# bikuta6/nbody-deep-sim

Measured on AMD Instinct MI355X. Metric: pair-interactions/sec, direct O(N^2) leapfrog N-body, fp32, higher is better.
Workload: dtype f32; 1 GPU; Plummer sphere, 65536 particles, direct all-pairs leapfrog step (BASELINE configs[1] shape: 65536 bodies per GPU); n_particles=65536, particles_per_gpu=65536, seed=1234, parallelism=single GPU

## Files before the change

include/nbd.h:

```cpp
#ifndef NBD_H_
#define NBD_H_

#include <stddef.h>
#include <stdint.h>

#ifdef __cplusplus
extern "C" {
#endif

#define NBD_ABI_VERSION 2
#define NBD_E_BADARG (-1)
#define NBD_E_WORKSPACE (-2)
#define NBD_E_UNSUPPORTED (-3)

#define NBD_SRC_PAD 64
#define NBD_CC_TILE 128
#define NBD_CC_GROUPS 8
#define NBD_CC_MAX_RES 4

typedef void* nbd_stream_t;

int nbd_abi_version(void);
size_t nbd_struct_size(const char* name);
const char* nbd_strerror(int code);
// ... 31 lines not shown
                                       float c_kick, void* workspace, size_t workspace_bytes, nbd_stream_t stream);

int nbd_kick_drift_f32(float* pos, float* vel, const float* acc, const float* mass, int n,
                       float c_kick, float c_drift, float* posm, nbd_stream_t stream);

int nbd_kick_f32(float* vel, const float* acc, int n, float c, nbd_stream_t stream);

int nbd_drift_f32(float* pos, const float* vel, int n, float c, nbd_stream_t stream);

int nbd_snapshot_f32(const float* pos, const float* vel, const float* acc, int n, float* out, nbd_stream_t stream);
int nbd_snapshot_f64(const double* pos, const double* vel, const double* acc, int n, double* out, nbd_stream_t stream);

size_t nbd_step_workspace_bytes(int n);

size_t nbd_step_workspace_pref_bytes(int n);

int nbd_leapfrog_step_f32(float* pos, float* vel, const float* acc_in, float* acc_out,
                          const float* mass, int n, float dt_half, float dt, float softening_sq,
                          float g_const, float* posm, void* workspace, size_t workspace_bytes,
                          nbd_stream_t stream);

int nbd_leapfrog_step_ev_f32(float* pos, float* vel, const float* acc_in, float* acc_out,
                             const float* mass, int n, float dt_half, float dt, float softening_sq,
                             float g_const, float* posm, void* workspace, size_t workspace_bytes,
                             nbd_stream_t stream, void* ev_force_begin, void* ev_force_end);
int nbd_leapfrog_step_uniform_f32(float* pos, float* vel, const float* acc_in, float* acc_out, const float* mass,
                                  float mass_value, int n, float dt_half, float dt, float softening_sq, float g_const,
                                  float* posm, void* workspace, size_t workspace_bytes, nbd_stream_t stream,
                                  void* ev_force_begin, void* ev_force_end);

size_t nbd_accel_sym_workspace_bytes(int n);
int nbd_accel_sym_uniform_f32(const float* posm, int n, float softening_sq, float g_const, float mass_value,
                              float* acc_out, void* workspace, size_t workspace_bytes, int variant, nbd_stream_t stream);

int nbd_euler_step_f32(float* pos, float* vel, float* acc_out, const float* mass, int n, float dt,
                       float softening_sq, float g_const, float* posm, void* workspace,
                       size_t workspace_bytes, nbd_stream_t stream);

size_t nbd_energy_workspace_bytes(int n);

int nbd_energy_f32(const float* posm, const float* vel, int n, float softening, float g_const,
                   double* out_uk, void* workspace, size_t workspace_bytes, nbd_stream_t stream);

size_t nbd_potential_workspace_bytes(int n_src, int n_tgt);
int nbd_potential_f32(const float* posm_src, int n_src, const float* posm_tgt, int n_tgt, int tgt_global_offset,
                      float softening_sq, float g_const, double* phi_out, void* workspace, size_t workspace_bytes,
                      nbd_stream_t stream);
int nbd_invariants_f64(const float* posm, const float* vel, const double* phi, int n, double* out_row,
                       nbd_stream_t stream);

int nbd_batch_plan(const int* offsets, int n_scenes, int* n_items, int* posm_rows, size_t* plan_bytes,
                   size_t* workspace_bytes);
int nbd_batch_plan_fill(const int* offsets, int n_scenes, void* plan, size_t plan_bytes);
int nbd_batch_pack_posm_f32(const int* offsets, int n_scenes, const void* plan, size_t plan_bytes, const float* pos,
                            const float* mass, float* posm, nbd_stream_t stream);
int nbd_batch_accel_f32(const int* offsets, int n_scenes, const void* plan, size_t plan_bytes, const float* pos,
                        const float* mass, const float* softening_sq, const float* g_const, float* acc_out,
                        float* posm, void* workspace, size_t workspace_bytes, nbd_stream_t stream);
int nbd_batch_leapfrog_step_f32(const int* offsets, int n_scenes, const void* plan, size_t plan_bytes, float* pos,
                                float* vel, const float* acc_in, float* acc_out, const float* mass, const float* dt_half,
                                const float* dt, const float* softening_sq, const float* g_const, float* posm,
                                void* workspace, size_t workspace_bytes, nbd_stream_t stream);
int nbd_batch_euler_step_f32(const int* offsets, int n_scenes, const void* plan, size_t plan_bytes, float* pos,
                             float* vel, float* acc_out, const float* mass, const float* dt, const float* softening_sq,
                             const float* g_const, float* posm, void* workspace, size_t workspace_bytes,
                             nbd_stream_t stream);
// ... 572 lines not shown
```

nbody-deep-sim_amd/csrc/direct_force.hip:

```cpp
#include <hip/hip_runtime.h>
#include <string.h>
#include <stdint.h>

#include <type_traits>

#include "../../include/nbd.h"
#include "direct_kernels.h"

namespace {

template <bool MASKED, int KU, bool UNI = false>
__global__ __launch_bounds__(64 * kWaves, KU == 4 ? 8 : 5) void accel_kernel(
    const f4* __restrict__ src, const SrcView sv, const f4* __restrict__ tgt,
    int n_tgt, int tgt_off, float eps2, float scale, float* __restrict__ out, int out_rows, int tile_len) {
  __shared__ f4 lds[kAccelLdsF4];
  const int tz = blockIdx.z * tile_len;
  const int t_base = blockIdx.x * kTgtPerWG;
  accel_body<KU, UNI>(src + tz, sv, std::integral_constant<bool, MASKED>{}, tgt + tz, n_tgt, tgt_off, t_base, blockIdx.y, eps2, scale, lds,
                      out + (size_t)tz * 3 + ((size_t)blockIdx.y * out_rows + t_base) * 3);
}

constexpr int kSymTile = 1024;
constexpr int kSymChunks = kSymTile / kChunk;
constexpr int kSymSlots = 16;
// ... 112 lines not shown
        const float v = (t & 1) ? v2.y : v2.x;
        float* o = o_own + t * 64 * 3 + comp;
        *o = init ? v : *o + v;
      }
    return;
  }
  __syncthreads();
  float* const mo = ldsf + (sg * 4 + tg) * 12 * 64;
#pragma unroll
  for (int t = 0; t < 4; ++t)
#pragma unroll
    for (int comp = 0; comp < 3; ++comp) {
      const f2 v2 = own[(t >> 1) * 3 + comp];
      mo[(comp * 4 + t) * 64 + lane] = (t & 1) ? v2.y : v2.x;
    }
  __syncthreads();
  if (sg != 0) return;
#pragma unroll
  for (int t = 0; t < 4; ++t)
#pragma unroll
    for (int comp = 0; comp < 3; ++comp) {
      const float* src = ldsf + tg * 12 * 64 + (comp * 4 + t) * 64 + lane;
      float v = src[0];
#pragma unroll
      for (int g = 1; g < SG; ++g) v += src[g * 4 * 12 * 64];
      float* o = o_own + t * 64 * 3 + comp;
      *o = init ? v : *o + v;
    }
}

constexpr int kSym2Pairs = kSymChunks / 2;
constexpr int kSym2T = 8;
constexpr int kSym2G = 2;

__global__ __launch_bounds__(512, 4) void accel_sym2_kernel(const f4* __restrict__ posm, int n, int m, int r0,
                                                            int n_slots, float eps2, float* __restrict__ out) {
  constexpr int kXyF = kSym2Pairs * 128 * 4;
  constexpr int kZF = kSym2Pairs * 128 * 2;
  constexpr int kReactF = 2 * 8 * 6 * 64;
  constexpr int kOwnF = 8 * 3 * kSym2T * 64;
  static_assert(kXyF + kZF + kReactF == kOwnF, "one 48-KiB LDS image");
  __shared__ f4 lds[kOwnF / 4];
  float* const ldsf = reinterpret_cast<float*>(lds);
  f4* const xy = lds;
  f2* const zz = reinterpret_cast<f2*>(ldsf + kXyF);
  float* const react = ldsf + kXyF + kZF;

  int ta, tb, slot;
  bool init;
  sym_round_match(blockIdx.x, m, r0, n_slots, ta, tb, slot, init);

  const int lane = threadIdx.x & 63;
  const int wave = __builtin_amdgcn_readfirstlane(threadIdx.x >> 6);
  const int tg = wave & 1, sg = wave >> 1;
  {
    const f4 u = posm[tb * kSymTile + wave * kChunk + lane];
    const f4 v = posm[tb * kSymTile + (wave + kSym2Pairs) * kChunk + lane];
    const f4 q = {u.x, v.x, u.y, v.y};
    const f2 z = {u.z, v.z};
    xy[wave * 128 + lane] = q; xy[wave * 128 + 64 + lane] = q;
    zz[wave * 128 + lane] = z; zz[wave * 128 + 64 + lane] = z;
  }
  const int row0 = ta * kSymTile + tg * 512 + lane;
  f2 txy[kSym2T], tzz[kSym2T / 2];
  f2 ax[kSym2T], ay[kSym2T], az[kSym2T];
#pragma unroll
  for (int t = 0; t < kSym2T; ++t) {
    const f4 q = posm[row0 + t * 64];
    txy[t] = f2{q.x, q.y};
    if (t & 1) tzz[t >> 1].y = q.z; else tzz[t >> 1].x = q.z;
    ax[t] = ay[t] = az[t] = f2{0.f, 0.f};
  }
  f2 e2 = {eps2, eps2};
  asm volatile("" : "+v"(e2));
  __syncthreads();

#pragma unroll 1
  for (int j = 0; j < 2; ++j) {
    const int p = sg * 2 + j;
    const f4* const bxy = xy + p * 128 + lane;
    const f2* const bz = zz + p * 128 + lane;
    f2 rx = {0.f, 0.f}, ry = {0.f, 0.f}, rz = {0.f, 0.f};
#pragma unroll 1
// ... 61 lines not shown
#pragma unroll
    for (int i = 0; i < 6; ++i) olda[i] = o_a[threadIdx.x + i * 512];
  }
  __syncthreads();

#pragma unroll
  for (int i = 0; i < 6; ++i) {
    const int o = threadIdx.x + i * 512;
    const int row = o / 3, comp = o - row * 3;
    const int c = row >> 6, l = row & 63, p = c & (kSym2Pairs - 1), hf = c / kSym2Pairs;
    const float* rs = react + ((p & 1) * 8 + (p >> 1) * 2) * 6 * 64 + (comp * 2 + hf) * 64 + l;
    const float v = rs[0] + rs[6 * 64];
    o_b[o] = init ? v : oldb[i] + v;
  }
  __syncthreads();
#pragma unroll
  for (int t = 0; t < kSym2T; ++t) {
    float* const mo = ldsf + ((sg * 2 + tg) * 3 * kSym2T + t) * 64 + lane;
    mo[0 * kSym2T * 64] = ax[t].x + ax[t].y;
    mo[1 * kSym2T * 64] = ay[t].x + ay[t].y;
    mo[2 * kSym2T * 64] = az[t].x + az[t].y;
  }
  __syncthreads();
#pragma unroll
  for (int i = 0; i < 6; ++i) {
    const int o = threadIdx.x + i * 512;
    const int row = o / 3, comp = o - row * 3;
    const int g = row >> 9, t = (row >> 6) & (kSym2T - 1), l = row & 63;
    const float* os = ldsf + ((g * 3 + comp) * kSym2T + t) * 64 + l;
    constexpr int kSg = 2 * 3 * kSym2T * 64;
    const float v = ((os[0] + os[kSg]) + os[2 * kSg]) + os[3 * kSg];
    o_a[o] = init ? v : olda[i] + v;
  }
}

__global__ __launch_bounds__(256) void finish_kernel(const float* __restrict__ slabs, int n_slabs,
                                                     size_t slab_stride, float g, float* __restrict__ acc,
                                                     float* __restrict__ vel, float c_kick, int n3) {
  __shared__ float part[4][64];
  const int lane = threadIdx.x & 63, w = threadIdx.x >> 6;
  const int i = blockIdx.x * 64 + lane;
  float sum = 0.f;
  if (i < n3)
    for (int s = w; s < n_slabs; s += 4) sum += slabs[s * slab_stride + i];
  part[w][lane] = sum;
  __syncthreads();
  if (w != 0 || i >= n3) return;
  const float a = __fmul_rn(g, (part[0][lane] + part[1][lane]) + (part[2][lane] + part[3][lane]));
  acc[i] = a;
  if (vel) vel[i] = __fadd_rn(vel[i], __fmul_rn(c_kick, a));
}

__global__ __launch_bounds__(256) void pack_kernel(const float* __restrict__ pos,
                                                   const float* __restrict__ mass, int n, int n_pad,
                                                   f4* __restrict__ posm) {
  const int i = blockIdx.x * 256 + threadIdx.x;
  if (i >= n_pad) return;
  f4 v = {0.f, 0.f, 0.f, 0.f};
  if (i < n) v = f4{pos[3 * i], pos[3 * i + 1], pos[3 * i + 2], mass[i]};
  posm[i] = v;
}

__global__ __launch_bounds__(256) void kick_drift_kernel(float* __restrict__ pos, float* __restrict__ vel,
                                                         const float* __restrict__ acc,
                                                         const float* __restrict__ mass, int n, int n_pad,
                                                         float ck, float cd, f4* __restrict__ posm) {
// ... 154 lines not shown
SymPlan plan_sym(int n, int slots_avail = 0) {
  SymPlan p;
  p.m = n / kSymTile;
  p.m &= ~1;
  p.core = p.m * kSymTile;
  p.rem = n - p.core;
  const int narrow = p.m < kSymSlots ? p.m : kSymSlots, wide = p.m < kSymSlotsCap ? p.m : kSymSlotsCap;
  const int avail = slots_avail - (p.rem > 0 ? 1 : 0);
  p.slots = avail < narrow ? narrow : (avail < wide ? avail : wide);
  p.total_slots = p.slots + (p.rem > 0 ? 1 : 0);
  return p;
}

size_t sym_workspace_bytes(int n) {
  const SymPlan p = plan_sym(n);
  return p.m < 2 ? 0 : (size_t)p.total_slots * n * 3 * sizeof(float);
}

int sym_slots_avail(int n, size_t workspace_bytes) {
  const size_t s = workspace_bytes / ((size_t)n * 3 * sizeof(float));
  return s > (size_t)kSymSlotsCap + 1 ? kSymSlotsCap + 1 : (int)s;
}

size_t sym_workspace_pref_bytes(int n) {
  const SymPlan p = plan_sym(n);
  if (p.m < 2) return 0;
  const int k = p.m < kSymSlotsPref ? p.m : kSymSlotsPref;
  return (size_t)(k + (p.rem > 0 ? 1 : 0)) * n * 3 * sizeof(float);
}

constexpr int kSymStepMinN = 65536;
bool sym_step(int n, float eps2) { return n >= kSymStepMinN && eps2 >= kEps2Masked; }

int launch_sym(const float* posm, int n, float eps2, float* slots, const SymPlan& sp, hipStream_t st, int variant = 0) {
  const f4* pm = reinterpret_cast<const f4*>(posm);
  const AccelPlan dp = make_plan(kSymTile / kTgtPerWG, 1, kSymChunks);
  int rc = launch_accel(posm, full_view(kSymTile, dp), posm, kSymTile, 0, eps2, 1.0f, slots, dp, st, true, n, sp.m,
                        kSymTile);
  if (rc) return rc;
  const int rounds = sp.m - 1;
  for (int r0 = 0; r0 < rounds;) {
    const int r1 = r0 == 0 ? (sp.slots - 1 < rounds ? sp.slots - 1 : rounds) : (r0 + sp.slots < rounds ? r0 + sp.slots : rounds);
    const int wgs = (r1 - r0) * (sp.m / 2);
    if (variant == 2) accel_sym2_kernel<<<wgs, 512, 0, st>>>(pm, n, sp.m, r0, sp.slots, eps2, slots);
    else if (variant == 1) accel_sym_kernel<2><<<wgs, 512, 0, st>>>(pm, n, sp.m, r0, sp.slots, eps2, slots);
    else accel_sym_kernel<4><<<wgs, 1024, 0, st>>>(pm, n, sp.m, r0, sp.slots, eps2, slots);
    if ((rc = launch_status())) return rc;
    r0 = r1;
  }
  if (sp.rem == 0) return 0;
  const AccelPlan tp = make_plan(ceil_div(sp.rem, kTgtPerWG), sp.total_slots, ceil_div(n, kChunk));
  rc = launch_accel(posm, full_view(n, tp), posm + (size_t)sp.core * 4, sp.rem, sp.core, eps2, 1.0f,
                    slots + (size_t)sp.core * 3, tp, st, true, n);
  if (rc) return rc;
  SrcView sv;
  const AccelPlan cp = make_plan(sp.core / kTgtPerWG, 1, excluded_view(n, 0, sp.core, &sv));
  return launch_accel(posm, sv, posm, sp.core, 0, eps2, 1.0f, slots + (size_t)sp.slots * n * 3, cp, st, true, n);
}

}

extern "C" {

int nbd_abi_version(void) { return NBD_ABI_VERSION; }

size_t nbd_struct_size(const char* name) {
  if (!name) return 0;
#define NBD_SZ(T) if (!strcmp(name, #T)) return sizeof(T);
  NBD_SZ(nbd_gnn_layer_args) NBD_SZ(nbd_gnn_forward_args) NBD_SZ(nbd_knn_pq_args) NBD_SZ(nbd_gnn_train_args)
  NBD_SZ(nbd_gnn_train_grads) NBD_SZ(nbd_cc_train_args) NBD_SZ(nbd_cc_train_grads) NBD_SZ(nbd_cc_pairs_job)
#undef NBD_SZ
  return 0;
}

// ... 18 lines not shown
}

size_t nbd_accel_workspace_bytes(int n_src, int n_tgt) {
  if (n_src <= 0 || n_tgt <= 0) return 0;
  const AccelPlan p = plan_accel(n_src, n_tgt);
  return p.slabs > 1 ? (size_t)p.slabs * n_tgt * 3 * sizeof(float) : 0;
}

int nbd_accel_plan(int n_src, int n_tgt, int* groups, int* slabs, int* chunks_per_wave) {
  if (n_src <= 0 || n_tgt <= 0) return NBD_E_BADARG;
  const AccelPlan p = plan_accel(n_src, n_tgt);
  if (groups) *groups = p.groups;
  if (slabs) *slabs = p.slabs;
  if (chunks_per_wave) *chunks_per_wave = p.cpw;
  return 0;
}

size_t nbd_step_workspace_bytes(int n) {
  if (n <= 0) return 0;
  const size_t all_pairs = (size_t)plan_accel(n, n).slabs * n * 3 * sizeof(float);
  const size_t sym = sym_step(n, kEps2Masked) ? sym_workspace_bytes(n) : 0;
  return sym > all_pairs ? sym : all_pairs;
}

size_t nbd_step_workspace_pref_bytes(int n) {
  if (n <= 0) return 0;
  const size_t least = nbd_step_workspace_bytes(n);
  const size_t pref = sym_step(n, kEps2Masked) ? sym_workspace_pref_bytes(n) : 0;
  return pref > least ? pref : least;
}

size_t nbd_accel_sym_workspace_bytes(int n) { return n <= 0 ? 0 : sym_workspace_bytes(n); }

int nbd_accel_sym_uniform_f32(const float* posm, int n, float softening_sq, float g_const, float mass_value,
                              float* acc_out, void* workspace, size_t workspace_bytes, int variant, nbd_stream_t stream) {
  if (n < 0 || (n > 0 && (!posm || !acc_out)) || misaligned16(posm) || variant < 0 || variant > 2) return NBD_E_BADARG;
  if (n == 0) return 0;
  if (plan_sym(n).m < 2 || softening_sq < kEps2Masked) return NBD_E_UNSUPPORTED;
  if (!workspace || workspace_bytes < sym_workspace_bytes(n)) return NBD_E_WORKSPACE;
  hipStream_t st = (hipStream_t)stream;
  float* slots = static_cast<float*>(workspace);
  const SymPlan sp = plan_sym(n, sym_slots_avail(n, workspace_bytes));
  int rc = launch_sym(posm, n, softening_sq, slots, sp, st, variant);
  if (rc) return rc;
  const int n3 = 3 * n;
  finish_kernel<<<ceil_div(n3, 64), 256, 0, st>>>(slots, sp.total_slots, (size_t)n3, g_const * mass_value,
                                                   acc_out, nullptr, 0.f, n3);
  return launch_status();
}

int nbd_accel_f32(const float* posm_src, int n_src, const float* posm_tgt, int n_tgt,
                  int tgt_global_offset, float softening_sq, float g_const, float* acc_out,
                  void* workspace, size_t workspace_bytes, nbd_stream_t stream) {
  if (n_src < 0 || n_tgt < 0) return NBD_E_BADARG;
  if (n_tgt == 0) return 0;
  if (!acc_out || !posm_tgt || misaligned16(posm_tgt)) return NBD_E_BADARG;
  hipStream_t st = (hipStream_t)stream;
  if (n_src == 0) {
    zero_f32_kernel<<<ceil_div(n_tgt * 3, 256), 256, 0, st>>>(acc_out, (size_t)n_tgt * 3);
    return launch_status();
  }
  if (!posm_src || misaligned16(posm_src)) return NBD_E_BADARG;
  const AccelPlan p = plan_accel(n_src, n_tgt);
  if (p.slabs == 1)
    return launch_accel(posm_src, full_view(n_src, p), posm_tgt, n_tgt, tgt_global_offset, softening_sq,
                        g_const, acc_out, p, st);
  const size_t need = (size_t)p.slabs * n_tgt * 3 * sizeof(float);
  if (!workspace || workspace_bytes < need) return NBD_E_WORKSPACE;
  float* slabs = static_cast<float*>(workspace);
  int rc = launch_accel(posm_src, full_view(n_src, p), posm_tgt, n_tgt, tgt_global_offset, softening_sq,
                        1.0f, slabs, p, st);
  if (rc) return rc;
  const int n3 = n_tgt * 3;
  finish_kernel<<<ceil_div(n3, 64), 256, 0, st>>>(slabs, p.slabs, (size_t)n3, g_const, acc_out,
                                                   nullptr, 0.f, n3);
  return launch_status();
}

size_t nbd_accel_tuned_workspace_bytes(int n_tgt, int slabs) {
  if (n_tgt <= 0 || slabs <= 0) return 0;
  return (size_t)slabs * n_tgt * 3 * sizeof(float);
// ... 148 lines not shown
int nbd_snapshot_f32(const float* pos, const float* vel, const float* acc, int n, float* out, nbd_stream_t stream) {
  if (n < 0 || (n > 0 && (!pos || !vel || !acc || !out))) return NBD_E_BADARG;
  if (n == 0) return 0;
  snapshot_kernel<float><<<ceil_div(3 * n, 256), 256, 0, (hipStream_t)stream>>>(pos, vel, acc, 3 * n, out);
  return launch_status();
}

int nbd_snapshot_f64(const double* pos, const double* vel, const double* acc, int n, double* out, nbd_stream_t stream) {
  if (n < 0 || (n > 0 && (!pos || !vel || !acc || !out))) return NBD_E_BADARG;
  if (n > 0 && ((reinterpret_cast<uintptr_t>(out) & 7) != 0)) return NBD_E_BADARG;
  if (n == 0) return 0;
  snapshot_kernel<double><<<ceil_div(3 * n, 256), 256, 0, (hipStream_t)stream>>>(pos, vel, acc, 3 * n, out);
  return launch_status();
}

static int step_force(float* pos, float* vel, const float* acc_in, float* acc_out, const float* mass, int n, bool euler,
                      float c_kick, float c_drift, float softening_sq, float g_scale, bool uniform, float* posm,
                      void* workspace, size_t workspace_bytes, nbd_stream_t stream, void* ev_force_begin,
                      void* ev_force_end) {
  if (n < 0) return NBD_E_BADARG;
  if (n == 0) return 0;
  if (!pos || !vel || (!euler && !acc_in) || !acc_out || !mass || !posm || misaligned16(posm)) return NBD_E_BADARG;
  hipStream_t st = (hipStream_t)stream;
  const bool sym = uniform && sym_step(n, softening_sq);
  const AccelPlan p = plan_accel(n, n);
  const size_t need = sym ? sym_workspace_bytes(n) : (size_t)p.slabs * n * 3 * sizeof(float);
  if (!workspace || workspace_bytes < need) return NBD_E_WORKSPACE;
  int rc = euler ? nbd_pack_posm_f32(pos, mass, n, posm, stream)
                 : nbd_kick_drift_f32(pos, vel, acc_in, mass, n, c_kick, c_drift, posm, stream);
  if (rc) return rc;
  float* slabs = static_cast<float*>(workspace);
  if (ev_force_begin && (rc = check(hipEventRecord((hipEvent_t)ev_force_begin, st)))) return rc;
  const SymPlan sp = plan_sym(n, sym ? sym_slots_avail(n, workspace_bytes) : 0);
  if (sym) rc = launch_sym(posm, n, softening_sq, slabs, sp, st, 2);
  else rc = launch_accel(posm, full_view(n, p), posm, n, 0, softening_sq, 1.0f, slabs, p, st, uniform);
  if (rc) return rc;
  if (ev_force_end && (rc = check(hipEventRecord((hipEvent_t)ev_force_end, st)))) return rc;
  const int n3 = 3 * n;
  const int n_slabs = sym ? sp.total_slots : p.slabs;
  finish_kernel<<<ceil_div(n3, 64), 256, 0, st>>>(slabs, n_slabs, (size_t)n3, g_scale, acc_out, vel, c_kick, n3);
  return launch_status();
}

int nbd_leapfrog_step_ev_f32(float* pos, float* vel, const float* acc_in, float* acc_out,
                          const float* mass, int n, float dt_half, float dt, float softening_sq,
                          float g_const, float* posm, void* workspace, size_t workspace_bytes,
                          nbd_stream_t stream, void* ev_force_begin, void* ev_force_end) {
  return step_force(pos, vel, acc_in, acc_out, mass, n, false, dt_half, dt, softening_sq, g_const, false, posm,
                    workspace, workspace_bytes, stream, ev_force_begin, ev_force_end);
}

int nbd_leapfrog_step_uniform_f32(float* pos, float* vel, const float* acc_in, float* acc_out, const float* mass,
                                  float mass_value, int n, float dt_half, float dt, float softening_sq, float g_const,
                                  float* posm, void* workspace, size_t workspace_bytes, nbd_stream_t stream,
                                  void* ev_force_begin, void* ev_force_end) {
  return step_force(pos, vel, acc_in, acc_out, mass, n, false, dt_half, dt, softening_sq, g_const * mass_value, true,
                    posm, workspace, workspace_bytes, stream, ev_force_begin, ev_force_end);
}

int nbd_leapfrog_step_f32(float* pos, float* vel, const float* acc_in, float* acc_out,
                          const float* mass, int n, float dt_half, float dt, float softening_sq,
                          float g_const, float* posm, void* workspace, size_t workspace_bytes,
                          nbd_stream_t stream) {
  return nbd_leapfrog_step_ev_f32(pos, vel, acc_in, acc_out, mass, n, dt_half, dt, softening_sq, g_const,
                                  posm, workspace, workspace_bytes, stream, nullptr, nullptr);
}

// ... 42 lines not shown
```

nbody-deep-sim_amd/csrc/direct_kernels.h:

```cpp
#pragma once
#include <hip/hip_runtime.h>
#include <stdint.h>

#include "../../include/nbd.h"

typedef float f2 __attribute__((ext_vector_type(2)));
typedef float f4 __attribute__((ext_vector_type(4)));
typedef double d4 __attribute__((ext_vector_type(4)));

#define GPTR(p) ((const __attribute__((address_space(1))) void*)(p))
#define LPTR(p) ((__attribute__((address_space(3))) void*)(p))

namespace {

constexpr int kWaves = 4;
constexpr int kTgtPerLane = 2;
constexpr int kTgtPerWG = 64 * kTgtPerLane;
constexpr int kChunk = NBD_SRC_PAD;
constexpr int kMaxSlabs = 64;
constexpr float kEps2Masked = 1e-24f;

__host__ __device__ inline int ceil_div(int a, int b) { return (a + b - 1) / b; }
inline bool misaligned16(const void* p) { return (reinterpret_cast<uintptr_t>(p) & 15) != 0; }
inline bool misaligned32(const void* p) { return (reinterpret_cast<uintptr_t>(p) & 31) != 0; }
// ... 74 lines not shown
                                               const f2 e2, f2& ax, f2& ay, f2& az) {
  f4 p[KU];
  f2 dx[KU], dy[KU], dz[KU], s[KU];
#pragma unroll
  for (int u = 0; u < KU; ++u) {
    p[u] = buf[u];
    if (UNI) asm("" : "+v"(p[u]));
    dx[u] = f2{p[u].x, p[u].x} - xi; dy[u] = f2{p[u].y, p[u].y} - yi; dz[u] = f2{p[u].z, p[u].z} - zi;
    f2 r2 = __builtin_elementwise_fma(dx[u], dx[u], e2);
    r2 = __builtin_elementwise_fma(dy[u], dy[u], r2);
    s[u] = __builtin_elementwise_fma(dz[u], dz[u], r2);
  }
#pragma unroll
  for (int u = 0; u < KU; ++u) s[u] = f2{__builtin_amdgcn_rsqf(s[u].x), __builtin_amdgcn_rsqf(s[u].y)};
  __builtin_amdgcn_sched_group_barrier(0x400, 2 * KU, 0);
#pragma unroll
  for (int u = 0; u < KU; ++u) {
    const f2 zm = {p[u].z, p[u].w};
    const f2 s3 = (s[u] * s[u]) * s[u];
    f2 w;
    if (UNI) w = s3;
    else asm("v_pk_mul_f32 %0, %1, %2 op_sel:[1,0] op_sel_hi:[1,1]" : "=v"(w) : "v"(zm), "v"(s3));
    ax = __builtin_elementwise_fma(w, dx[u], ax);
    ay = __builtin_elementwise_fma(w, dy[u], ay);
    az = __builtin_elementwise_fma(w, dz[u], az);
  }
}

constexpr int kAccelLdsF4 = kWaves * 2 * kChunk + kWaves * 6 * 64 / 4;

template <int KU, bool UNI, class Masked>
__device__ __forceinline__ void accel_body(const f4* __restrict__ src, const SrcView& sv, const Masked masked,
                                           const f4* __restrict__ tgt, int n_tgt, int tgt_off, int t_base, int slab,
                                           float eps2, float scale, f4* lds, float* __restrict__ dst) {
  const int lane = threadIdx.x & 63;
  const int wave = __builtin_amdgcn_readfirstlane(threadIdx.x >> 6);
  const int i0 = t_base + lane, i1 = t_base + 64 + lane;
  const f4 t0 = tgt[min(i0, n_tgt - 1)], t1 = tgt[min(i1, n_tgt - 1)];
  const f2 xi = {t0.x, t1.x}, yi = {t0.y, t1.y}, zi = {t0.z, t1.z};
  f2 ax = {0.f, 0.f}, ay = {0.f, 0.f}, az = {0.f, 0.f};
  f2 e2 = {eps2, eps2};
  asm volatile("" : "+v"(e2));

  const int jw = slab * kWaves + wave;
  const int c_begin = jw * sv.cpw_q + min(jw, sv.cpw_r), c_end = c_begin + sv.cpw_q + (jw < sv.cpw_r ? 1 : 0);
  f4* stage = &lds[wave * 2 * kChunk];
  const f4* s_lane = src + lane;
  auto phys = [&](int c) { return c + (c >= sv.skip_c0 ? sv.skip_cn : 0); };
  if (c_begin < c_end)
    __builtin_amdgcn_global_load_lds(GPTR(s_lane + (size_t)phys(c_begin) * kChunk), LPTR(stage), 16, 0, 0);
  for (int c = c_begin; c < c_end; ++c) {
    const int b = (c - c_begin) & 1;
    if (c + 1 < c_end) {
      __builtin_amdgcn_global_load_lds(GPTR(s_lane + (size_t)phys(c + 1) * kChunk),
                                       LPTR(stage + (b ^ 1) * kChunk), 16, 0, 0);
      asm volatile("s_waitcnt vmcnt(1)" ::: "memory");
    } else {
      asm volatile("s_waitcnt vmcnt(0)" ::: "memory");
    }
    const f4* buf = stage + b * kChunk;
    const int pc = phys(c);
    const int j0 = pc * kChunk;
    if (masked || pc == sv.edge0 || pc == sv.edge1 || (UNI && pc == sv.tail)) {
#pragma unroll 4
      for (int j = 0; j < kChunk; ++j)
        interact<true, UNI>(buf[j], xi, yi, zi, e2, ax, ay, az, j0 + j, tgt_off + i0, tgt_off + i1, sv);
    } else {
#pragma unroll 1
      for (int j = 0; j < kChunk; j += KU) interact_block<KU, UNI>(buf + j, xi, yi, zi, e2, ax, ay, az);
    }
  }

  float* red = reinterpret_cast<float*>(&lds[kWaves * 2 * kChunk]);
  float* mine = red + wave * 6 * 64;
  mine[0 * 64 + lane] = ax.x; mine[1 * 64 + lane] = ax.y;
  mine[2 * 64 + lane] = ay.x; mine[3 * 64 + lane] = ay.y;
  mine[4 * 64 + lane] = az.x; mine[5 * 64 + lane] = az.y;
  __syncthreads();
  const int n_valid = min(kTgtPerWG, n_tgt - t_base) * 3;
  for (int o = threadIdx.x; o < n_valid; o += 64 * kWaves) {
    const int lt = o / 3, comp = o - lt * 3;
    const int idx = (comp * 2 + (lt >> 6)) * 64 + (lt & 63);
    float sum = red[idx];
#pragma unroll
    for (int w = 1; w < kWaves; ++w) sum += red[w * 6 * 64 + idx];
    dst[o] = __fmul_rn(scale, sum);
  }
}

template <bool MASKED>
__device__ __forceinline__ void energy_pair(const f4 p, const f2 xi, const f2 yi, const f2 zi, const f2 soft,
                                            f2& u, int j, int i0, int i1, int n) {
  const f2 dx = f2{p.x, p.x} - xi, dy = f2{p.y, p.y} - yi, dz = f2{p.z, p.z} - zi;
  f2 d2 = dx * dx;
  d2 = __builtin_elementwise_fma(dy, dy, d2);
  d2 = __builtin_elementwise_fma(dz, dz, d2);
  const f2 den = f2{__builtin_amdgcn_sqrtf(d2.x), __builtin_amdgcn_sqrtf(d2.y)} + soft;
  const f2 inv = {__builtin_amdgcn_rcpf(den.x), __builtin_amdgcn_rcpf(den.y)};
  f2 t = f2{p.w, p.w} * inv;
  if (MASKED) {
    t.x = (j > i0 && j < n) ? t.x : 0.f;
    t.y = (j > i1 && j < n) ? t.y : 0.f;
  }
  u += t;
}

constexpr int kEnergyLdsF4 = kWaves * 2 * kChunk + 8;

__device__ __forceinline__ void energy_body(const f4* __restrict__ posm, int n, int n_chunks, int t_base, int slab,
                                            int slabs, float soft_, const bool all_masked, f4* lds,
                                            double* __restrict__ dst) {
  const int lane = threadIdx.x & 63;
  const int wave = __builtin_amdgcn_readfirstlane(threadIdx.x >> 6);
  const int i0 = t_base + lane, i1 = t_base + 64 + lane;
  const f4 t0 = posm[min(i0, n - 1)], t1 = posm[min(i1, n - 1)];
  const f2 xi = {t0.x, t1.x}, yi = {t0.y, t1.y}, zi = {t0.z, t1.z};
  f2 u = {0.f, 0.f};
  f2 soft = {soft_, soft_};
  asm volatile("" : "+v"(soft));
  const int c_lo = t_base / kChunk;
// ... 156 lines not shown
```

nbody-deep-sim_amd/nbd/_lib.py:

```python
from __future__ import annotations

import ctypes
import os
import subprocess
from ctypes import c_char_p, c_double, c_float, c_int, c_int64, c_size_t, c_void_p, POINTER

import torch

_HERE = os.path.dirname(os.path.abspath(__file__))
CSRC_DIR = os.path.normpath(os.path.join(_HERE, "..", "csrc"))
LIB_PATH = os.environ.get("NBD_LIB_OVERRIDE") or os.path.join(CSRC_DIR, "libnbd_hip.so")


class NbdError(RuntimeError):
    pass


class NbdUnsupported(NbdError):
    """A configuration a fast path does not cover (NBD_E_UNSUPPORTED, or the Python-side check in front of it): callers that
    probe a path catch THIS and fall back; any other NbdError is a real failure and propagates."""


def build(verbose: bool = False) -> str:
    res = subprocess.run(["make", "-C", CSRC_DIR, "-j4"], capture_output=True, text=True)
# ... 93 lines not shown
                              c_void_p, c_size_t, c_void_p]),
    "nbd_accel_tuned_workspace_bytes": (c_size_t, [c_int, c_int]),
    "nbd_accel_tuned_f32": (c_int, [c_void_p, c_int, c_int, c_int, c_void_p, c_int, c_int, c_float, c_float,
                                    c_void_p, c_void_p, c_size_t, c_int, c_int, c_void_p]),
    "nbd_shard_plan": (c_int, [c_int, c_int, c_int, POINTER(c_int), POINTER(c_int), POINTER(c_int),
                               POINTER(c_int)]),
    "nbd_shard_workspace_bytes": (c_size_t, [c_int, c_int, c_int]),
    "nbd_shard_force_local_f32": (c_int, [c_void_p, c_int, c_float, c_void_p, c_size_t, c_int, c_int, c_void_p]),
    "nbd_shard_force_remote_f32": (c_int, [c_void_p, c_int, c_void_p, c_int, c_int, c_float, c_float, c_void_p,
                                           c_void_p, c_float, c_void_p, c_size_t, c_void_p]),
    "nbd_shard_force_local_uniform_f32": (c_int, [c_void_p, c_int, c_float, c_void_p, c_size_t, c_int, c_int, c_void_p]),
    "nbd_shard_force_remote_uniform_f32": (c_int, [c_void_p, c_int, c_void_p, c_int, c_int, c_float, c_float, c_float,
                                                   c_void_p, c_void_p, c_float, c_void_p, c_size_t, c_void_p]),
    "nbd_kick_drift_f32": (c_int, [c_void_p, c_void_p, c_void_p, c_void_p, c_int, c_float, c_float,
                                   c_void_p, c_void_p]),
    "nbd_kick_f32": (c_int, [c_void_p, c_void_p, c_int, c_float, c_void_p]),
    "nbd_drift_f32": (c_int, [c_void_p, c_void_p, c_int, c_float, c_void_p]),
    "nbd_snapshot_f32": (c_int, [c_void_p, c_void_p, c_void_p, c_int, c_void_p, c_void_p]),
    "nbd_snapshot_f64": (c_int, [c_void_p, c_void_p, c_void_p, c_int, c_void_p, c_void_p]),
    "nbd_step_workspace_bytes": (c_size_t, [c_int]),
    "nbd_step_workspace_pref_bytes": (c_size_t, [c_int]),
    "nbd_leapfrog_step_f32": (c_int, [c_void_p, c_void_p, c_void_p, c_void_p, c_void_p, c_int,
                                      c_float, c_float, c_float, c_float, c_void_p, c_void_p,
                                      c_size_t, c_void_p]),
    "nbd_leapfrog_step_ev_f32": (c_int, [c_void_p, c_void_p, c_void_p, c_void_p, c_void_p, c_int,
                                         c_float, c_float, c_float, c_float, c_void_p, c_void_p,
                                         c_size_t, c_void_p, c_void_p, c_void_p]),
    "nbd_leapfrog_step_uniform_f32": (c_int, [c_void_p, c_void_p, c_void_p, c_void_p, c_void_p, c_float, c_int,
                                              c_float, c_float, c_float, c_float, c_void_p, c_void_p,
                                              c_size_t, c_void_p, c_void_p, c_void_p]),
    "nbd_accel_sym_workspace_bytes": (c_size_t, [c_int]),
    "nbd_accel_sym_uniform_f32": (c_int, [c_void_p, c_int, c_float, c_float, c_float, c_void_p, c_void_p, c_size_t,
                                          c_int, c_void_p]),
    "nbd_euler_step_f32": (c_int, [c_void_p, c_void_p, c_void_p, c_void_p, c_int, c_float, c_float,
                                   c_float, c_void_p, c_void_p, c_size_t, c_void_p]),
    "nbd_energy_workspace_bytes": (c_size_t, [c_int]),
    "nbd_energy_f32": (c_int, [c_void_p, c_void_p, c_int, c_float, c_float, c_void_p, c_void_p,
                               c_size_t, c_void_p]),
    "nbd_potential_workspace_bytes": (c_size_t, [c_int, c_int]),
    "nbd_potential_f32": (c_int, [c_void_p, c_int, c_void_p, c_int, c_int, c_float, c_float, c_void_p, c_void_p,
                                  c_size_t, c_void_p]),
    "nbd_invariants_f64": (c_int, [c_void_p, c_void_p, c_void_p, c_int, c_void_p, c_void_p]),
    "nbd_batch_potential_f32": (c_int, [c_void_p, c_int, c_void_p, c_size_t, c_void_p, c_void_p, c_void_p, c_void_p,
                                        c_void_p, c_size_t, c_void_p]),
    "nbd_batch_invariants_f64": (c_int, [c_void_p, c_int, c_void_p, c_size_t, c_void_p, c_void_p, c_void_p, c_void_p,
                                         c_void_p]),
    "nbd_batch_plan": (c_int, [c_void_p, c_int, POINTER(c_int), POINTER(c_int), POINTER(c_size_t), POINTER(c_size_t)]),
    "nbd_batch_plan_fill": (c_int, [c_void_p, c_int, c_void_p, c_size_t]),
    "nbd_batch_pack_posm_f32": (c_int, [c_void_p, c_int, c_void_p, c_size_t, c_void_p, c_void_p, c_void_p, c_void_p]),
    "nbd_batch_accel_f32": (c_int, [c_void_p, c_int, c_void_p, c_size_t, c_void_p, c_void_p, c_void_p, c_void_p,
                                    c_void_p, c_void_p, c_void_p, c_size_t, c_void_p]),
    "nbd_batch_leapfrog_step_f32": (c_int, [c_void_p, c_int, c_void_p, c_size_t, c_void_p, c_void_p, c_void_p, c_void_p,
                                            c_void_p, c_void_p, c_void_p, c_void_p, c_void_p, c_void_p, c_void_p, c_size_t,
                                            c_void_p]),
    "nbd_batch_euler_step_f32": (c_int, [c_void_p, c_int, c_void_p, c_size_t, c_void_p, c_void_p, c_void_p, c_void_p,
                                         c_void_p, c_void_p, c_void_p, c_void_p, c_void_p, c_size_t, c_void_p]),
    "nbd_batch_energies": (c_int, [c_void_p, c_int, c_void_p, c_size_t, c_void_p, c_void_p, c_void_p, c_void_p, c_void_p,
                                   c_void_p, c_size_t, c_void_p]),
    "nbd_batch_hermite_workspace_bytes": (c_int, [c_void_p, c_int, POINTER(c_size_t)]),
    "nbd_batch_accel_jerk_f32": (c_int, [c_void_p, c_int, c_void_p, c_size_t, c_void_p, c_void_p, c_void_p, c_void_p,
                                         c_void_p, c_void_p, c_void_p, c_void_p, c_void_p, c_size_t, c_void_p]),
    "nbd_batch_hermite_step_f32": (c_int, [c_void_p, c_int, c_void_p, c_size_t, c_void_p, c_void_p, c_void_p, c_void_p,
                                           c_void_p, c_void_p, c_void_p, c_void_p, c_void_p, c_void_p, c_void_p, c_void_p,
                                           c_size_t, c_void_p]),
    "nbd_batch_f64_plan": (c_int, [c_void_p, c_int, POINTER(c_int), POINTER(c_int), POINTER(c_size_t)]),
    "nbd_batch_f64_workspace_bytes": (c_int, [c_void_p, c_int, POINTER(c_size_t)]),
# ... 357 lines not shown
```

Before: 6747 billion pair-interactions/s.

## Fuse diagonal self-tiles and all symmetric tile-pair rounds into one launch

Adds a tail kernel that, when the slot count equals the tile count, runs every symmetric tile-pair work group and the diagonal self-tile accel work in a single launch. The diagonal tiles are handled by packing two 256-thread accel_body halves into each 512-thread block, with each half using its own LDS region. This removes the separate diagonal launch and the multi-round sym2 launches, along with the tail imbalance and launch gaps between them. The leapfrog step now uses this variant by default, and accel_body gains an explicit thread-id parameter.

After: 6831 billion pair-interactions/s, median of 6. +1.2%, better.

```diff
diff --git a/include/nbd.h b/include/nbd.h
--- a/include/nbd.h
+++ b/include/nbd.h
@@ -87,6 +87,8 @@
 size_t nbd_accel_sym_workspace_bytes(int n);
 int nbd_accel_sym_uniform_f32(const float* posm, int n, float softening_sq, float g_const, float mass_value,
                               float* acc_out, void* workspace, size_t workspace_bytes, int variant, nbd_stream_t stream);
+int nbd_accel_sym_tail_uniform_f32(const float* posm, int n, float softening_sq, float g_const, float mass_value,
+                                   float* acc_out, void* workspace, size_t workspace_bytes, nbd_stream_t stream);
 
 int nbd_euler_step_f32(float* pos, float* vel, float* acc_out, const float* mass, int n, float dt,
                        float softening_sq, float g_const, float* posm, void* workspace,
diff --git a/nbody-deep-sim_amd/csrc/direct_force.hip b/nbody-deep-sim_amd/csrc/direct_force.hip
--- a/nbody-deep-sim_amd/csrc/direct_force.hip
+++ b/nbody-deep-sim_amd/csrc/direct_force.hip
@@ -168,15 +168,16 @@
 constexpr int kSym2Pairs = kSymChunks / 2;
 constexpr int kSym2T = 8;
 constexpr int kSym2G = 2;
-
-__global__ __launch_bounds__(512, 4) void accel_sym2_kernel(const f4* __restrict__ posm, int n, int m, int r0,
-                                                            int n_slots, float eps2, float* __restrict__ out) {
-  constexpr int kXyF = kSym2Pairs * 128 * 4;
-  constexpr int kZF = kSym2Pairs * 128 * 2;
-  constexpr int kReactF = 2 * 8 * 6 * 64;
-  constexpr int kOwnF = 8 * 3 * kSym2T * 64;
-  static_assert(kXyF + kZF + kReactF == kOwnF, "one 48-KiB LDS image");
-  __shared__ f4 lds[kOwnF / 4];
+constexpr int kSym2XyF = kSym2Pairs * 128 * 4;
+constexpr int kSym2ZF = kSym2Pairs * 128 * 2;
+constexpr int kSym2ReactF = 2 * 8 * 6 * 64;
+constexpr int kSym2OwnF = 8 * 3 * kSym2T * 64;
+static_assert(kSym2XyF + kSym2ZF + kSym2ReactF == kSym2OwnF, "one 48-KiB LDS image");
+constexpr int kSym2LdsF4 = kSym2OwnF / 4;
+
+__device__ __forceinline__ void sym2_body(const f4* __restrict__ posm, int n, int m, int r0, int n_slots, int wg,
+                                          float eps2, float* __restrict__ out, f4* lds) {
+  constexpr int kXyF = kSym2XyF, kZF = kSym2ZF;
   float* const ldsf = reinterpret_cast<float*>(lds);
   f4* const xy = lds;
   f2* const zz = reinterpret_cast<f2*>(ldsf + kXyF);
@@ -184,7 +185,7 @@
 
   int ta, tb, slot;
   bool init;
-  sym_round_match(blockIdx.x, m, r0, n_slots, ta, tb, slot, init);
+  sym_round_match(wg, m, r0, n_slots, ta, tb, slot, init);
 
   const int lane = threadIdx.x & 63;
   const int wave = __builtin_amdgcn_readfirstlane(threadIdx.x >> 6);
@@ -312,6 +313,30 @@
     const float v = ((os[0] + os[kSg]) + os[2 * kSg]) + os[3 * kSg];
     o_a[o] = init ? v : olda[i] + v;
   }
+}
+
+__global__ __launch_bounds__(512, 4) void accel_sym2_kernel(const f4* __restrict__ posm, int n, int m, int r0,
+                                                            int n_slots, float eps2, float* __restrict__ out) {
+  __shared__ f4 lds[kSym2LdsF4];
+  sym2_body(posm, n, m, r0, n_slots, blockIdx.x, eps2, out, lds);
+}
+
+__global__ __launch_bounds__(512, 4) void accel_sym2_tail_kernel(const f4* __restrict__ posm, int n, int m, float eps2,
+                                                                 float* __restrict__ out) {
+  __shared__ f4 lds[kSym2LdsF4];
+  static_assert(2 * kAccelLdsF4 <= kSym2LdsF4, "two accel_body regions in the tile-pair image");
+  const int pairs = (m >> 1) * (m - 1);
+  if ((int)blockIdx.x < pairs) {
+    sym2_body(posm, n, m, 0, m, blockIdx.x, eps2, out, lds);
+    return;
+  }
+  const int half = __builtin_amdgcn_readfirstlane(threadIdx.x >> 8);
+  const int g = ((int)blockIdx.x - pairs) * 2 + half;
+  constexpr int kGroups = kSymTile / kTgtPerWG;
+  const int tz = (g / kGroups) * kSymTile, t_base = (g % kGroups) * kTgtPerWG;
+  const SrcView sv = full_view(kSymTile, kSymChunks, 1);
+  accel_body<8, true>(posm + tz, sv, std::false_type{}, posm + tz, kSymTile, 0, t_base, 0, eps2, 1.0f,
+                      lds + half * kAccelLdsF4, out + ((size_t)tz + t_base) * 3, (int)(threadIdx.x & 255));
 }
 
 __global__ __launch_bounds__(256) void finish_kernel(const float* __restrict__ slabs, int n_slabs,
@@ -532,14 +557,24 @@
 constexpr int kSymStepMinN = 65536;
 bool sym_step(int n, float eps2) { return n >= kSymStepMinN && eps2 >= kEps2Masked; }
 
+constexpr int kSymTailVariant = 3;
 int launch_sym(const float* posm, int n, float eps2, float* slots, const SymPlan& sp, hipStream_t st, int variant = 0) {
   const f4* pm = reinterpret_cast<const f4*>(posm);
-  const AccelPlan dp = make_plan(kSymTile / kTgtPerWG, 1, kSymChunks);
-  int rc = launch_accel(posm, full_view(kSymTile, dp), posm, kSymTile, 0, eps2, 1.0f, slots, dp, st, true, n, sp.m,
-                        kSymTile);
-  if (rc) return rc;
+  const bool tail = variant == kSymTailVariant && sp.slots == sp.m;
+  if (variant == kSymTailVariant) variant = 2;
+  int rc = 0;
+  if (tail) {
+    accel_sym2_tail_kernel<<<(sp.m / 2) * (sp.m - 1) + sp.m * (kSymTile / kTgtPerWG) / 2, 512, 0, st>>>(pm, n, sp.m,
+                                                                                                      eps2, slots);
+    if ((rc = launch_status())) return rc;
+  } else {
+    const AccelPlan dp = make_plan(kSymTile / kTgtPerWG, 1, kSymChunks);
+    rc = launch_accel(posm, full_view(kSymTile, dp), posm, kSymTile, 0, eps2, 1.0f, slots, dp, st, true, n, sp.m,
+                      kSymTile);
+    if (rc) return rc;
+  }
   const int rounds = sp.m - 1;
-  for (int r0 = 0; r0 < rounds;) {
+  for (int r0 = tail ? rounds : 0; r0 < rounds;) {
     const int r1 = r0 == 0 ? (sp.slots - 1 < rounds ? sp.slots - 1 : rounds) : (r0 + sp.slots < rounds ? r0 + sp.slots : rounds);
     const int wgs = (r1 - r0) * (sp.m / 2);
     if (variant == 2) accel_sym2_kernel<<<wgs, 512, 0, st>>>(pm, n, sp.m, r0, sp.slots, eps2, slots);
@@ -624,9 +659,9 @@
 
 size_t nbd_accel_sym_workspace_bytes(int n) { return n <= 0 ? 0 : sym_workspace_bytes(n); }
 
-int nbd_accel_sym_uniform_f32(const float* posm, int n, float softening_sq, float g_const, float mass_value,
-                              float* acc_out, void* workspace, size_t workspace_bytes, int variant, nbd_stream_t stream) {
-  if (n < 0 || (n > 0 && (!posm || !acc_out)) || misaligned16(posm) || variant < 0 || variant > 2) return NBD_E_BADARG;
+static int accel_sym_uniform(const float* posm, int n, float softening_sq, float g_const, float mass_value,
+                             float* acc_out, void* workspace, size_t workspace_bytes, int variant, nbd_stream_t stream) {
+  if (n < 0 || (n > 0 && (!posm || !acc_out)) || misaligned16(posm)) return NBD_E_BADARG;
   if (n == 0) return 0;
   if (plan_sym(n).m < 2 || softening_sq < kEps2Masked) return NBD_E_UNSUPPORTED;
   if (!workspace || workspace_bytes < sym_workspace_bytes(n)) return NBD_E_WORKSPACE;
@@ -639,6 +674,19 @@
   finish_kernel<<<ceil_div(n3, 64), 256, 0, st>>>(slots, sp.total_slots, (size_t)n3, g_const * mass_value,
                                                    acc_out, nullptr, 0.f, n3);
   return launch_status();
+}
+
+int nbd_accel_sym_uniform_f32(const float* posm, int n, float softening_sq, float g_const, float mass_value,
+                              float* acc_out, void* workspace, size_t workspace_bytes, int variant, nbd_stream_t stream) {
+  if (variant < 0 || variant > 2) return NBD_E_BADARG;
+  return accel_sym_uniform(posm, n, softening_sq, g_const, mass_value, acc_out, workspace, workspace_bytes, variant,
+                           stream);
+}
+
+int nbd_accel_sym_tail_uniform_f32(const float* posm, int n, float softening_sq, float g_const, float mass_value,
+                                   float* acc_out, void* workspace, size_t workspace_bytes, nbd_stream_t stream) {
+  return accel_sym_uniform(posm, n, softening_sq, g_const, mass_value, acc_out, workspace, workspace_bytes,
+                           kSymTailVariant, stream);
 }
 
 int nbd_accel_f32(const float* posm_src, int n_src, const float* posm_tgt, int n_tgt,
@@ -853,7 +901,7 @@
   float* slabs = static_cast<float*>(workspace);
   if (ev_force_begin && (rc = check(hipEventRecord((hipEvent_t)ev_force_begin, st)))) return rc;
   const SymPlan sp = plan_sym(n, sym ? sym_slots_avail(n, workspace_bytes) : 0);
-  if (sym) rc = launch_sym(posm, n, softening_sq, slabs, sp, st, 2);
+  if (sym) rc = launch_sym(posm, n, softening_sq, slabs, sp, st, kSymTailVariant);
   else rc = launch_accel(posm, full_view(n, p), posm, n, 0, softening_sq, 1.0f, slabs, p, st, uniform);
   if (rc) return rc;
   if (ev_force_end && (rc = check(hipEventRecord((hipEvent_t)ev_force_end, st)))) return rc;
diff --git a/nbody-deep-sim_amd/csrc/direct_kernels.h b/nbody-deep-sim_amd/csrc/direct_kernels.h
--- a/nbody-deep-sim_amd/csrc/direct_kernels.h
+++ b/nbody-deep-sim_amd/csrc/direct_kernels.h
@@ -130,9 +130,9 @@
 template <int KU, bool UNI, class Masked>
 __device__ __forceinline__ void accel_body(const f4* __restrict__ src, const SrcView& sv, const Masked masked,
                                            const f4* __restrict__ tgt, int n_tgt, int tgt_off, int t_base, int slab,
-                                           float eps2, float scale, f4* lds, float* __restrict__ dst) {
-  const int lane = threadIdx.x & 63;
-  const int wave = __builtin_amdgcn_readfirstlane(threadIdx.x >> 6);
+                                           float eps2, float scale, f4* lds, float* __restrict__ dst, const int tid) {
+  const int lane = tid & 63;
+  const int wave = __builtin_amdgcn_readfirstlane(tid >> 6);
   const int i0 = t_base + lane, i1 = t_base + 64 + lane;
   const f4 t0 = tgt[min(i0, n_tgt - 1)], t1 = tgt[min(i1, n_tgt - 1)];
   const f2 xi = {t0.x, t1.x}, yi = {t0.y, t1.y}, zi = {t0.z, t1.z};
@@ -176,7 +176,7 @@
   mine[4 * 64 + lane] = az.x; mine[5 * 64 + lane] = az.y;
   __syncthreads();
   const int n_valid = min(kTgtPerWG, n_tgt - t_base) * 3;
-  for (int o = threadIdx.x; o < n_valid; o += 64 * kWaves) {
+  for (int o = tid; o < n_valid; o += 64 * kWaves) {
     const int lt = o / 3, comp = o - lt * 3;
     const int idx = (comp * 2 + (lt >> 6)) * 64 + (lt & 63);
     float sum = red[idx];
@@ -184,6 +184,13 @@
     for (int w = 1; w < kWaves; ++w) sum += red[w * 6 * 64 + idx];
     dst[o] = __fmul_rn(scale, sum);
   }
+}
+
+template <int KU, bool UNI, class Masked>
+__device__ __forceinline__ void accel_body(const f4* __restrict__ src, const SrcView& sv, const Masked masked,
+                                           const f4* __restrict__ tgt, int n_tgt, int tgt_off, int t_base, int slab,
+                                           float eps2, float scale, f4* lds, float* __restrict__ dst) {
+  accel_body<KU, UNI>(src, sv, masked, tgt, n_tgt, tgt_off, t_base, slab, eps2, scale, lds, dst, threadIdx.x);
 }
 
 template <bool MASKED>
diff --git a/nbody-deep-sim_amd/nbd/_lib.py b/nbody-deep-sim_amd/nbd/_lib.py
--- a/nbody-deep-sim_amd/nbd/_lib.py
+++ b/nbody-deep-sim_amd/nbd/_lib.py
@@ -149,6 +149,8 @@
     "nbd_accel_sym_workspace_bytes": (c_size_t, [c_int]),
     "nbd_accel_sym_uniform_f32": (c_int, [c_void_p, c_int, c_float, c_float, c_float, c_void_p, c_void_p, c_size_t,
                                           c_int, c_void_p]),
+    "nbd_accel_sym_tail_uniform_f32": (c_int, [c_void_p, c_int, c_float, c_float, c_float, c_void_p, c_void_p,
+                                               c_size_t, c_void_p]),
     "nbd_euler_step_f32": (c_int, [c_void_p, c_void_p, c_void_p, c_void_p, c_int, c_float, c_float,
                                    c_float, c_void_p, c_void_p, c_size_t, c_void_p]),
     "nbd_energy_workspace_bytes": (c_size_t, [c_int]),
```
